# ChangUk/RecommenderSystems

Hardware: AMD Instinct MI355X
Metric: RWR seeds/sec + achieved HBM GB/s on 100M-edge bipartite graph, 1/2/4/8 GPUs (higher is better)
Workload: dtype f64

## Files before the change

### recommendersystems_amd/csrc/iterate.hip

```cpp
#include "iterate.h"

#include <climits>
#include <cstdlib>
#include <type_traits>

namespace rwr {

template <int G, bool VF>
__global__ __launch_bounds__(256) void k_spmm(int32_t n, const int64_t *__restrict__ in_ptr,
                                              const int32_t *__restrict__ in_src,
                                              const double *__restrict__ in_w,
                                              const int32_t *__restrict__ row_order, int32_t nrows,
                                              const double *__restrict__ X, double *__restrict__ Y,
                                              const int32_t *__restrict__ seeds, double c1, int skip_seed_row,
                                              const double *__restrict__ w_src, double *__restrict__ Zout)
{
    constexpr int RPW = WAVE / G;
    constexpr int U = 4;
    const int tile = blockIdx.y;
    const size_t toff = (size_t)tile * (size_t)n * G;
    X += toff;
    Y += toff;
    if (VF && Zout) Zout += toff;
    const int lane = threadIdx.x & (WAVE - 1);
    const int sub = lane / G, k = lane % G;
    const int32_t my_seed = skip_seed_row ? seeds[tile * G + k] : -1;
    const int wpb = blockDim.x / WAVE;
    const int64_t nwaves = (int64_t)gridDim.x * wpb;
    for (int64_t rb = ((int64_t)blockIdx.x * wpb + threadIdx.x / WAVE) * RPW; rb < nrows; rb += nwaves * RPW) {
        const int64_t r = rb + sub;
        int32_t j = -1;
        int64_t p = 0, e = 0;
        if (r < nrows) {
            j = row_order[r];
            p = in_ptr[j];
            e = in_ptr[j + 1];
        }
        double acc = 0.0;
        for (; p + U <= e; p += U) {
            int32_t idx[U];
            double wv[U], xv[U];
#pragma unroll
            for (int u = 0; u < U; ++u) idx[u] = in_src[p + u];
#pragma unroll
            for (int u = 0; u < U; ++u) wv[u] = VF ? 0.0 : in_w[p + u];
#pragma unroll
            for (int u = 0; u < U; ++u) xv[u] = X[(size_t)idx[u] * G + k];
#pragma unroll
            for (int u = 0; u < U; ++u) {
                if (VF) {
                    acc += xv[u];
                } else {
                    double rw = c1 * xv[u];
                    acc += rw * wv[u];
                }
            }
        }
        for (; p < e; ++p) {
            if (VF) {
                acc += X[(size_t)in_src[p] * G + k];
            } else {
                double rw = c1 * X[(size_t)in_src[p] * G + k];
                acc += rw * in_w[p];
            }
        }
        if (j >= 0 && j != my_seed) {
            Y[(size_t)j * G + k] = acc;
            if (VF && Zout) { const double rw = c1 * acc; Zout[(size_t)j * G + k] = rw * w_src[j]; }
        }
    }
}

template <int G, int CH, bool CHECK, bool WRITE, bool VF>
__device__ __forceinline__ void spmm_chunked_body(int32_t n, const int64_t *__restrict__ in_ptr,
                                                  const int32_t *__restrict__ in_src,
                                                  const double *__restrict__ in_w,
                                                  const int32_t *__restrict__ row_order, int32_t nrows,
                                                  const double *__restrict__ X, double *__restrict__ Y,
                                                  const int32_t *__restrict__ seeds, double c1,
                                                  int skip_seed_row, const uint32_t *__restrict__ nz_in,
                                                  uint32_t *__restrict__ nz_out,
                                                  const uint32_t *__restrict__ act,
                                                  const double *__restrict__ w_src, double *__restrict__ Zout)
{
    static_assert(G >= 8 && G <= 64, "chunked SpMM needs 8 <= G <= 64");
    constexpr int RPW = WAVE / G;
    const int tile = blockIdx.y;
    const size_t toff = (size_t)tile * (size_t)n * G;
    X += toff;
    Y += toff;
    if (VF && Zout) Zout += toff;
    const size_t nzw = ((size_t)n + 31) / 32;
    if (CHECK) nz_in += (size_t)tile * nzw;
    if (WRITE) nz_out += (size_t)tile * nzw;
    if (CHECK && act) act += (size_t)tile * nzw;
    const int lane = threadIdx.x & (WAVE - 1);
    const int sub = lane / G, k = lane % G;
    const int gbase = (lane - k) << 2;
    const int32_t my_seed = skip_seed_row ? seeds[tile * G + k] : -1;
    const int wpb = blockDim.x / WAVE;
    const int64_t nwaves = (int64_t)gridDim.x * wpb;
    for (int64_t rb = ((int64_t)blockIdx.x * wpb + threadIdx.x / WAVE) * RPW; rb < nrows; rb += nwaves * RPW) {
        const int64_t r = rb + sub;
        int32_t j = -1;
        int64_t p = 0, e = 0;
        if (r < nrows) {
            j = row_order[r];
            p = in_ptr[j];
            e = in_ptr[j + 1];
            if (CHECK && act && !((act[(uint32_t)j >> 5] >> (j & 31)) & 1u)) e = p;
        }
        double acc = 0.0;
        while (__any(p < e)) {
            const int64_t left = e - p;
            const int cnt = left > CH ? CH : (left > 0 ? (int)left : 0);
            int32_t my_idx = 0;
            double my_w = 0.0;
            if (k < cnt) {
                my_idx = in_src[p + k];
                if (!VF) my_w = in_w[p + k];
                if (CHECK) {
                    const uint32_t wd = nz_in[(uint32_t)my_idx >> 5];
                    if (!((wd >> (my_idx & 31)) & 1u)) my_idx |= (int32_t)0x80000000;
                }
            }
            const int wlo = __double2loint(my_w), whi = __double2hiint(my_w);
            if (CHECK) {
                const unsigned long long lm = __ballot(k < cnt && my_idx >= 0);
                unsigned long long um = lm;
                if (G < 64) {
#pragma unroll
                    for (int sh = G; sh < 64; sh <<= 1) um |= um >> sh;
                    um &= (1ull << (G & 63)) - 1ull;
                }
                if (__popcll(um) <= 4) {
                    while (um) {
                        const int t = __builtin_ctzll(um);
                        um &= um - 1;
                        const int idx = __builtin_amdgcn_ds_bpermute(gbase + (t << 2), my_idx);
                        if (VF) {
                            if (t < cnt && idx >= 0) acc += X[(size_t)idx * G + k];
                        } else {
                            const int lo = __builtin_amdgcn_ds_bpermute(gbase + (t << 2), wlo);
                            const int hi = __builtin_amdgcn_ds_bpermute(gbase + (t << 2), whi);
                            if (t < cnt && idx >= 0) {
                                const double rw = c1 * X[(size_t)idx * G + k];
                                acc += rw * __hiloint2double(hi, lo);
                            }
                        }
                    }
                    p += cnt;
                    continue;
                }
            }
            double xv[CH], wv[CH];
#pragma unroll
            for (int t = 0; t < CH; ++t) {
                const int idx = __builtin_amdgcn_ds_bpermute(gbase + (t << 2), my_idx);
                if (!VF) {
                    const int lo = __builtin_amdgcn_ds_bpermute(gbase + (t << 2), wlo);
                    const int hi = __builtin_amdgcn_ds_bpermute(gbase + (t << 2), whi);
                    wv[t] = __hiloint2double(hi, lo);
                }
                xv[t] = (t < cnt && idx >= 0) ? X[(size_t)idx * G + k] : 0.0;
            }
#pragma unroll
            for (int t = 0; t < CH; ++t) {
                if (t < cnt) {
                    if (VF) {
                        acc += xv[t];
                    } else {
                        double rw = c1 * xv[t];
                        acc += rw * wv[t];
                    }
                }
            }
            p += cnt;
        }
        if (j >= 0 && j != my_seed) {
            Y[(size_t)j * G + k] = acc;
            if (VF && Zout) { const double rw = c1 * acc; Zout[(size_t)j * G + k] = rw * w_src[j]; }
        }
        if (WRITE) {
            const unsigned long long nzb = __ballot(acc != 0.0);
            const unsigned long long gmask = (G == 64) ? ~0ull : (((1ull << (G & 63)) - 1ull) << (sub * G));
            if (k == 0 && j >= 0 && (nzb & gmask)) atomicOr(&nz_out[(uint32_t)j >> 5], 1u << (j & 31));
        }
    }
}

template <int G, int CH, bool CHECK, bool WRITE, bool VF, bool LIST>
__global__ __launch_bounds__(256) void k_spmm_chunked(int32_t n, const int64_t *__restrict__ in_ptr,
                                                      const int32_t *__restrict__ in_src,
                                                      const double *__restrict__ in_w,
                                                      const int32_t *__restrict__ row_order, int32_t nrows,
                                                      const double *__restrict__ X, double *__restrict__ Y,
                                                      const int32_t *__restrict__ seeds, double c1,
                                                      int skip_seed_row, const uint32_t *__restrict__ nz_in,
                                                      uint32_t *__restrict__ nz_out,
                                                      const uint32_t *__restrict__ act,
                                                      const double *__restrict__ w_src, double *__restrict__ Zout)
{
    spmm_chunked_body<G, CH, CHECK, WRITE, VF>(n, in_ptr, in_src, in_w, row_order, nrows, X, Y, seeds, c1, skip_seed_row,
                                               nz_in, nz_out, act, w_src, Zout);
}

template <int G, int CH, bool VF>
__global__ __launch_bounds__(256) void k_spmm_frontier(int32_t n, const int64_t *__restrict__ in_ptr,
                                                       const int32_t *__restrict__ in_src,
                                                       const double *__restrict__ in_w,
                                                       const int32_t *__restrict__ fl_rows,
                                                       const int32_t *__restrict__ fl_cnt,
                                                       const double *__restrict__ X, double *__restrict__ Y,
                                                       const int32_t *__restrict__ seeds, double c1,
                                                       int skip_seed_row, const uint32_t *__restrict__ nz_in,
                                                       uint32_t *__restrict__ nz_out,
                                                       const double *__restrict__ w_src, double *__restrict__ Zout)
{
    const int tile = blockIdx.y;
    spmm_chunked_body<G, CH, true, true, VF>(n, in_ptr, in_src, in_w, fl_rows + (size_t)tile * (size_t)n, fl_cnt[tile], X, Y,
                                             seeds, c1, skip_seed_row, nz_in, nz_out, nullptr, w_src, Zout);
}

__global__ __launch_bounds__(256) void k_mark_active(int32_t n, const uint32_t *__restrict__ nz, uint32_t *__restrict__ act,
                                                     const int64_t *__restrict__ rowptr, const int32_t *__restrict__ dst,
                                                     const uint8_t *__restrict__ etype, int G, const int32_t *__restrict__ seeds,
                                                     int32_t *__restrict__ fl_rows, int32_t *__restrict__ fl_cnt)
{
    const size_t nzw = ((size_t)n + 31) / 32;
    const int tile = blockIdx.y;
    const int lane = threadIdx.x & (WAVE - 1);
    const size_t wi = (size_t)blockIdx.x * (blockDim.x / WAVE) + threadIdx.x / WAVE;
    uint32_t *a = act + (size_t)tile * nzw;
    int32_t *list = fl_rows ? fl_rows + (size_t)tile * (size_t)n : nullptr;
    if (list && blockIdx.x == 0 && threadIdx.x < (unsigned)G) {
        const int32_t sr = seeds[tile * G + threadIdx.x];
        if (sr >= 0) {
            const uint32_t bit = 1u << (sr & 31);
            if (!(atomicOr(&a[(uint32_t)sr >> 5], bit) & bit)) list[atomicAdd(&fl_cnt[tile], 1)] = sr;
        }
    }
    if (wi >= nzw) return;
    uint32_t w = nz[(size_t)tile * nzw + wi];
    while (w) {
        const int b = __builtin_ctz(w);
        w &= w - 1;
        const int64_t i = (int64_t)wi * 32 + b;
        const int64_t p1 = rowptr[i + 1];
        if (!list) {
            for (int64_t p = rowptr[i] + lane; p < p1; p += WAVE)
                if (etype[p] != RWR_EDGE_UNDEFINED) {
                    const int32_t t = dst[p];
                    atomicOr(&a[(uint32_t)t >> 5], 1u << (t & 31));
                }
            continue;
        }
        for (int64_t p0 = rowptr[i]; p0 < p1; p0 += WAVE) {
            const int64_t p = p0 + lane;
            bool add = false;
            int32_t t = 0;
            if (p < p1 && etype[p] != RWR_EDGE_UNDEFINED) {
                t = dst[p];
                const uint32_t bit = 1u << (t & 31);
                add = !(atomicOr(&a[(uint32_t)t >> 5], bit) & bit);
            }
            const unsigned long long m = __ballot(add);
            if (!m) continue;
            const int leader = __builtin_ctzll(m);
            int base = 0;
            if (lane == leader) base = atomicAdd(&fl_cnt[tile], (int)__popcll(m));
            base = __shfl(base, leader);
            const int below = __builtin_amdgcn_mbcnt_hi((uint32_t)(m >> 32), __builtin_amdgcn_mbcnt_lo((uint32_t)m, 0u));
            if (add) list[base + below] = t;
        }
    }
}

template <int G>
__global__ __launch_bounds__(64) void k_seed_chain(int32_t n, int ntiles, const int64_t *__restrict__ in_ptr,
                                                   const int32_t *__restrict__ in_src,
                                                   const double *__restrict__ in_w,
                                                   const uint8_t *__restrict__ dangling,
                                                   const double *__restrict__ X, double *__restrict__ Y,
                                                   const int32_t *__restrict__ seeds, double c1,
                                                   uint32_t *__restrict__ nz_out)
{
    constexpr int U = 8;
    const int q = blockIdx.x * blockDim.x + threadIdx.x;
    if (q >= ntiles * G) return;
    const int tile = q / G, k = q % G;
    const int32_t s = seeds[q];
    if (s < 0) return;
    const double *x = X + (size_t)tile * (size_t)n * G + k;
    int64_t p = in_ptr[s];
    const int64_t e = in_ptr[s + 1];
    int32_t nxt = (p < e) ? in_src[p] : INT_MAX;
    double acc = 0.0;
    int32_t i = 0;
    for (; i + U <= n; i += U) {
        double xv[U];
        uint8_t dg[U];
#pragma unroll
        for (int u = 0; u < U; ++u) xv[u] = x[(size_t)(i + u) * G];
#pragma unroll
        for (int u = 0; u < U; ++u) dg[u] = dangling[i + u];
#pragma unroll
        for (int u = 0; u < U; ++u) {
            double rw = c1 * xv[u];
            while (nxt == i + u) {
                acc += rw * in_w[p];
                ++p;
                nxt = (p < e) ? in_src[p] : INT_MAX;
            }
            acc += dg[u] ? xv[u] : (xv[u] - rw);
        }
    }
    for (; i < n; ++i) {
        double xi = x[(size_t)i * G];
        double rw = c1 * xi;
        while (nxt == i) {
            acc += rw * in_w[p];
            ++p;
            nxt = (p < e) ? in_src[p] : INT_MAX;
        }
        acc += dangling[i] ? xi : (xi - rw);
    }
    Y[(size_t)tile * (size_t)n * G + (size_t)s * G + k] = acc;
    if (nz_out && acc != 0.0)
        atomicOr(&nz_out[(size_t)tile * (((size_t)n + 31) / 32) + ((uint32_t)s >> 5)], 1u << (s & 31));
}

__global__ void k_gate(const unsigned int *__restrict__ gate, unsigned int expected)
{
    const long long t0 = __builtin_amdgcn_s_memrealtime();
    while (__hip_atomic_load(gate, __ATOMIC_RELAXED, __HIP_MEMORY_SCOPE_AGENT) < expected) {
        if (__builtin_amdgcn_s_memrealtime() - t0 > 100000) break;
        __builtin_amdgcn_s_sleep(32);
    }
}

template <int G, bool VF>
__global__ __launch_bounds__(256) void k_seed_terms(int32_t n, const int64_t *__restrict__ in_ptr,
                                                    const int32_t *__restrict__ in_src,
                                                    const double *__restrict__ in_w, const double *__restrict__ X,
                                                    const int32_t *__restrict__ seeds, double c1,
                                                    const int64_t *__restrict__ evoff, double *__restrict__ evterm,
                                                    const uint32_t *__restrict__ nz)
{
    const int slot = blockIdx.y;
    const int32_t s = seeds[slot];
    if (s < 0) return;
    const int tile = slot / G, k = slot % G;
    const double *x = X + (size_t)tile * (size_t)n * G + k;
    const int64_t p0 = in_ptr[s], deg = in_ptr[s + 1] - p0;
    double *out = evterm + evoff[slot];
    if (nz) nz += (size_t)tile * (((size_t)n + 31) / 32);
    for (int64_t q = (int64_t)blockIdx.x * blockDim.x + threadIdx.x; q < deg; q += (int64_t)gridDim.x * blockDim.x) {
        const int32_t i = in_src[p0 + q];
        if (nz && !((nz[(uint32_t)i >> 5] >> (i & 31)) & 1u)) {
            out[q] = 0.0;
        } else if (VF) {
            out[q] = x[(size_t)i * G];
        } else {
            const double rw = c1 * x[(size_t)i * G];
            out[q] = rw * in_w[p0 + q];
        }
    }
}

template <int G>
__global__ __launch_bounds__(64) void k_seed_chain_sparse(int32_t n, const int64_t *__restrict__ in_ptr,
                                                          const int32_t *__restrict__ in_src,
                                                          const uint8_t *__restrict__ dangling,
                                                          const double *__restrict__ X, double *__restrict__ Y,
                                                          const int32_t *__restrict__ seeds, double c1,
                                                          const int64_t *__restrict__ evoff,
                                                          const double *__restrict__ evterm,
                                                          const uint32_t *__restrict__ nz_x, uint32_t *__restrict__ nz_out,
                                                          unsigned int *__restrict__ gate)
{
    if (threadIdx.x == 0 && gate) __hip_atomic_fetch_add(gate, 1u, __ATOMIC_RELAXED, __HIP_MEMORY_SCOPE_AGENT);
    const int tile = blockIdx.x, lane = threadIdx.x;
    const size_t nzw = ((size_t)n + 31) / 32;
    const uint32_t *bits = nz_x + (size_t)tile * nzw;
    const double *x = X + (size_t)tile * (size_t)n * G;
    const bool consumer = lane < G;
    const int k = lane % G;
    int32_t s = -1;
    int64_t p = 0, e = 0;
    const double *termp = evterm;
    if (consumer) {
        s = seeds[tile * G + k];
        if (s >= 0) {
            p = in_ptr[s];
            e = in_ptr[s + 1];
            termp = evterm + evoff[tile * G + k] - p;
        }
    }
    double acc = 0.0;
    for (size_t w0 = 0; w0 < nzw; w0 += WAVE) {
        const uint32_t word = (w0 + lane < nzw) ? bits[w0 + lane] : 0u;
        unsigned long long mask = __ballot(word != 0u);
        while (mask) {
            const int l = __builtin_ctzll(mask);
            mask &= mask - 1;
            uint32_t wv = (uint32_t)__builtin_amdgcn_readlane((int)word, l);
            while (wv) {
                const int b = __builtin_ctz(wv);
                wv &= wv - 1;
                const int32_t i = (int32_t)((w0 + l) * 32 + b);
                if (consumer && s >= 0) {
                    while (p < e && in_src[p] < i) ++p;
                    while (p < e && in_src[p] == i) { acc += termp[p]; ++p; }
                    const double xi = x[(size_t)i * G + k];
                    const double rw = c1 * xi;
                    acc += dangling[i] ? xi : (xi - rw);
                }
            }
        }
    }
    if (consumer && s >= 0) {
        Y[(size_t)tile * (size_t)n * G + (size_t)s * G + k] = acc;
        if (nz_out && acc != 0.0)
            atomicOr(&nz_out[(size_t)tile * nzw + ((uint32_t)s >> 5)], 1u << (s & 31));
    }
}

constexpr int CH3_NSW = 6;
constexpr int CH3_NST = CH3_NSW * WAVE;
constexpr int CH3_LPT = 16;
constexpr int CH3_CE = CH3_NST * CH3_LPT;
template <int G>
__global__ __launch_bounds__(WAVE + CH3_NST) void k_seed_chain_roles(
    int32_t n, const int64_t *__restrict__ in_ptr, const int32_t *__restrict__ in_src,
    const uint8_t *__restrict__ dangling, const double *__restrict__ X, double *__restrict__ Y,
    const int32_t *__restrict__ seeds, double c1, const int64_t *__restrict__ evoff,
    const double *__restrict__ evterm, uint32_t *__restrict__ nz_out, unsigned int *__restrict__ gate)
{
    if (threadIdx.x == 0 && gate) __hip_atomic_fetch_add(gate, 1u, __ATOMIC_RELAXED, __HIP_MEMORY_SCOPE_AGENT);
    constexpr int CR = CH3_CE / G;
    static_assert(CR % 32 == 0, "chunk rows must be a multiple of 32");
    extern __shared__ double rr[];
    const int tile = blockIdx.x;
    const double *x = X + (size_t)tile * (size_t)n * G;
    const int tid = threadIdx.x;
    const int64_t total = (int64_t)n * G;
    const int nchunks = (int)((total + CH3_CE - 1) / CH3_CE);

    if (tid >= WAVE) {
        const int st = tid - WAVE;
        double rega[CH3_LPT], regb[CH3_LPT];
        uint8_t dga[CH3_LPT], dgb[CH3_LPT];
#define CH3_LOAD(R, D, C)                                                       \
    {                                                                           \
        const int64_t base__ = (int64_t)(C) * CH3_CE;                           \
        _Pragma("unroll") for (int u = 0; u < CH3_LPT; ++u) {                   \
            int64_t el = base__ + (int64_t)u * CH3_NST + st;                    \
            el = el < total ? el : total - 1;                                   \
            R[u] = x[el];                                                       \
            D[u] = dangling[el / G];                                            \
        }                                                                       \
    }
#define CH3_STAGE(R, D, C)                                                                              \
    {                                                                                                   \
        const int64_t base__ = (int64_t)(C) * CH3_CE;                                                   \
        double *buf__ = rr + (size_t)((C) & 1) * CH3_CE;                                                \
        _Pragma("unroll") for (int u = 0; u < CH3_LPT; ++u) {                                           \
            const int off = u * CH3_NST + st;                                                           \
            const double xv = (base__ + off < total) ? R[u] : 0.0;   \
            const double rw = c1 * xv;                                                                  \
            buf__[off] = D[u] ? xv : (xv - rw);                                                         \
        }                                                                                               \
    }
        CH3_LOAD(rega, dga, 0)
        if (nchunks > 1) CH3_LOAD(regb, dgb, 1)
        for (int c = 0; c < nchunks; c += 2) {
            CH3_STAGE(rega, dga, c)
            if (c + 2 < nchunks) CH3_LOAD(rega, dga, c + 2)
            __builtin_amdgcn_fence(__ATOMIC_RELEASE, "workgroup", "local");
            __builtin_amdgcn_s_barrier();
            if (c + 1 < nchunks) {
                CH3_STAGE(regb, dgb, c + 1)
                if (c + 3 < nchunks) CH3_LOAD(regb, dgb, c + 3)
                __builtin_amdgcn_fence(__ATOMIC_RELEASE, "workgroup", "local");
                __builtin_amdgcn_s_barrier();
            }
        }
#undef CH3_LOAD
#undef CH3_STAGE
        return;
    }

    const bool consumer = tid < G;
    const int k = tid % G;
    int32_t s = -1;
    int64_t p = 0, e = 0;
    const int32_t *srcp = in_src;
    const double *termp = evterm;
    int32_t nxt = INT_MAX, raw_s = INT_MAX;
    double tcur = 0.0, raw_t = 0.0;
    bool has2 = false;
    if (consumer) {
        s = seeds[tile * G + k];
        if (s >= 0) {
            p = in_ptr[s];
            e = in_ptr[s + 1];
            termp = evterm + evoff[tile * G + k] - p;
            if (p < e) { nxt = srcp[p]; tcur = termp[p]; ++p; }
            if (p < e) { raw_s = srcp[p]; raw_t = termp[p]; has2 = true; ++p; }
        }
    }
    double acc = 0.0;
    __builtin_amdgcn_s_setprio(3);
    for (int c = 0; c < nchunks; ++c) {
        __builtin_amdgcn_s_barrier();
        __builtin_amdgcn_fence(__ATOMIC_ACQUIRE, "workgroup", "local");
        const double *buf = rr + (size_t)(c & 1) * CH3_CE;
        const int64_t row0 = (int64_t)c * CR;
#define CH3_READ(V, R0) _Pragma("unroll") for (int u = 0; u < 32; ++u) V[u] = buf[((R0) + u) * G + k];
#define CH3_FOLD(V, R0)                                                                                     \
    {                                                                                                       \
        const bool evt = __any(consumer && nxt < row0 + (R0) + 32);                                         \
        if (!evt) {                                                                                         \
            _Pragma("unroll") for (int u = 0; u < 32; ++u) acc += V[u];                                     \
        } else {                                                                                            \
            _Pragma("unroll") for (int u = 0; u < 32; ++u) {                                                \
                const int32_t i = (int32_t)(row0 + (R0)) + u;                                               \
                if (__any(consumer && nxt == i)) {                                                          \
                    while (consumer && nxt == i) {                                                          \
                        acc += tcur;                                                                        \
                        nxt = has2 ? raw_s : INT_MAX;  \
                        tcur = raw_t;                                                                       \
                        has2 = p < e;                 \
                        const int64_t pc = has2 ? p : e - 1;                                                \
                        raw_s = srcp[pc];                                                                   \
                        raw_t = termp[pc];                                                                  \
                        p += has2 ? 1 : 0;                                                                  \
                    }                                                                                       \
                }                                                                                           \
                acc += V[u];                            \
            }                                                                                               \
        }                                                                                                   \
    }
        double ra[32], rb[32];
        CH3_READ(ra, 0)
#pragma unroll 1
        for (int r0 = 0; r0 + 64 <= CR; r0 += 64) {
            CH3_READ(rb, r0 + 32)
            CH3_FOLD(ra, r0)
            if (r0 + 64 < CR) CH3_READ(ra, r0 + 64)
            CH3_FOLD(rb, r0 + 32)
        }
        if (CR % 64 != 0) CH3_FOLD(ra, CR - 32)
#undef CH3_READ
#undef CH3_FOLD
    }
    __builtin_amdgcn_s_setprio(0);
    if (consumer && s >= 0) {
        Y[(size_t)tile * (size_t)n * G + (size_t)s * G + k] = acc;
        if (nz_out && acc != 0.0)
            atomicOr(&nz_out[(size_t)tile * (((size_t)n + 31) / 32) + ((uint32_t)s >> 5)], 1u << (s & 31));
    }
}

__global__ void k_init_seeds(int32_t n, int ntiles, int G, double *__restrict__ X,
                             const int32_t *__restrict__ seeds, uint32_t *__restrict__ nz,
                             double *__restrict__ Z = nullptr, const double *__restrict__ w_src = nullptr, double c1 = 0.0)
{
    const int q = blockIdx.x * blockDim.x + threadIdx.x;
    if (q >= ntiles * G) return;
    const int32_t s = seeds[q];
    if (s < 0) return;
    const int tile = q / G;
    const size_t row = (size_t)tile * (size_t)n * G + (size_t)s * G;
    const double rw = c1 * (double)n;
    const double zs = Z ? rw * w_src[s] : 0.0;
    for (int kk = 0; kk < G; ++kk) {
        const bool mine = seeds[tile * G + kk] == s;
        X[row + kk] = mine ? (double)n : 0.0;
        if (Z) Z[row + kk] = mine ? zs : 0.0;
    }
    if (nz) atomicOr(&nz[(size_t)tile * (((size_t)n + 31) / 32) + ((uint32_t)s >> 5)], 1u << (s & 31));
}

__global__ void k_seed_z(int32_t n, int ntiles, int G, const double *__restrict__ Y, double *__restrict__ Z,
                         const int32_t *__restrict__ seeds, const double *__restrict__ w_src, double c1)
{
    const int q = blockIdx.x * blockDim.x + threadIdx.x;
    if (q >= ntiles * G) return;
    const int32_t s = seeds[q];
    if (s < 0) return;
    const size_t at = (size_t)(q / G) * (size_t)n * G + (size_t)s * G + (q % G);
    const double rw = c1 * Y[at];
    Z[at] = rw * w_src[s];
}
__global__ __launch_bounds__(256) void k_make_z(int64_t elems, int G, const double *__restrict__ X, double *__restrict__ Z,
                                                const double *__restrict__ w_src, double c1)
{
    const int64_t q = (int64_t)blockIdx.x * blockDim.x + threadIdx.x;
    if (q >= elems) return;
    const double rw = c1 * X[q];
    Z[q] = rw * w_src[q / G];
}

__global__ __launch_bounds__(256) void k_make_z_nz(int32_t lo, int32_t hi, int G, const double *__restrict__ X, double *__restrict__ Zs,
                                                   const double *__restrict__ w_src, double c1, uint32_t *__restrict__ nz)
{
    const int64_t j = ((int64_t)lo & ~(int64_t)63) + (int64_t)blockIdx.x * blockDim.x + threadIdx.x;
    bool any = false;
    if (j >= lo && j < hi) {
        const double w = w_src[j];
        const size_t at = (size_t)(j - lo) * G;
        for (int k = 0; k < G; ++k) {
            const double xv = X[(size_t)j * G + k];
            const double rw = c1 * xv;
            Zs[at + k] = rw * w;
            any = any || xv != 0.0;
        }
    }
    const unsigned long long m = __ballot(any);
    const int lane = threadIdx.x & (WAVE - 1);
    if (lane == 0 && (uint32_t)m) nz[(uint64_t)j >> 5] = (uint32_t)m;
    if (lane == 32 && (uint32_t)(m >> 32)) nz[(uint64_t)j >> 5] = (uint32_t)(m >> 32);
}


static PlanInput read_plan_knobs()
{
    PlanInput v;
    const char *e;
    if ((e = getenv("RWR_SPMM"))) v.spmm = atoi(e);
    if ((e = RWR_TUNE_ENV("RWR_NZ_ITERS"))) v.nz_iters = atoi(e);
    if ((e = getenv("RWR_ACT_ITERS"))) v.act_iters = atoi(e);
    if ((e = RWR_TUNE_ENV("RWR_ACT_MIN_N"))) v.act_min_n = atol(e);
    if ((e = getenv("RWR_FRONTIER_LIST"))) v.frontier_list = atoi(e);
    if ((e = getenv("RWR_CHAIN"))) v.chain = atoi(e);
    if ((e = RWR_TUNE_ENV("RWR_SCAN_WORK"))) v.scan_work = atof(e);
    if ((e = RWR_TUNE_ENV("RWR_SCAN_SIDE"))) v.scan_side = atoi(e);
    if ((e = RWR_TUNE_ENV("RWR_GATE"))) v.gate = atoi(e);
    if ((e = getenv("RWR_TAIL_ROWS"))) v.tail_rows = atoi(e);
    if ((e = RWR_TUNE_ENV("RWR_CHAIN_SERIAL"))) v.two_streams = atoi(e) == 0;
    return v;
}
static const PlanInput &plan_knobs() { static const PlanInput k = read_plan_knobs(); return k; }

template <class F> static void bool_dispatch(F &&f) { f(); }
template <class F, class... B> static void bool_dispatch(F &&f, bool b, B... bs)
{
    bool_dispatch([&](auto... c) { if (b) f(std::true_type{}, c...); else f(std::false_type{}, c...); }, bs...);
}

template <int G>
static void launch_spmm_g(rwr_graph *g, int tg, const SpmmArgs &a, hipStream_t s)
{
    const bool vf = a.Zin != nullptr;
    const double *GS = vf ? a.Zin : a.X;
    const int skip = a.skip_seed_row;
    constexpr int RPW = WAVE / G;
    constexpr int CH = G > 16 ? 16 : G;
    if constexpr (G >= 8) {
        if (a.rows.kind == Rows::Frontier) {
            const int32_t *fl_rows = g->fl_rows.p, *fl_cnt = g->fl_rows.p + (size_t)tg * (size_t)g->n;
            const unsigned want = cdiv((size_t)g->n / 10 + 1, (size_t)RPW * 4);
            const unsigned gx = want < 1u ? 1u : want < 2048u ? want : 2048u;
            bool_dispatch([&](auto v) {
                hipLaunchKernelGGL((k_spmm_frontier<G, CH, decltype(v)::value>), dim3(gx, tg), dim3(256), 0, s, g->n, g->in_ptr.p,
                                   g->in_src.p, g->in_w.p, fl_rows, fl_cnt, GS, a.Y, a.seeds, a.c1, skip, a.nz_in, a.nz_out,
                                   g->w_src.p, a.Zout);
            }, vf);
            return;
        }
    }
    const bool listed = a.rows.kind == Rows::Tail;
    const int32_t *order = listed ? g->tail_rows[a.rows.level].p : g->row_order.p;
    const int32_t nrows = listed ? g->tail_n[a.rows.level] : g->n;
    unsigned want = cdiv((size_t)nrows, (size_t)RPW * 4);
    unsigned gx = want < 1u ? 1u : want < 8192u ? want : 8192u;
    if constexpr (G == 1) {
        if (tg == 1 && plan_knobs().spmm != 0) {
            launch_spmv_exact(g, a.X, a.Y, a.seeds, a.c1, skip, a.act, a.nz_out, s, a.Zin, a.Zout, a.hub_scan);
            return;
        }
    }
    if constexpr (G >= 8) {
        if (plan_knobs().spmm != 0) {
            bool_dispatch([&](auto chk, auto wr, auto v, auto lst) {
                if constexpr (decltype(chk)::value || !decltype(wr)::value)
                    hipLaunchKernelGGL((k_spmm_chunked<G, CH, decltype(chk)::value, decltype(wr)::value, decltype(v)::value,
                                                       decltype(lst)::value>), dim3(gx, tg), dim3(256), 0, s, g->n, g->in_ptr.p,
                                       g->in_src.p, g->in_w.p, order, nrows, GS, a.Y, a.seeds, a.c1, skip, a.nz_in, a.nz_out,
                                       a.act, g->w_src.p, a.Zout);
            }, a.nz_in != nullptr, a.nz_in && a.nz_out, vf, listed);
            return;
        }
    }
    bool_dispatch([&](auto v) {
        hipLaunchKernelGGL((k_spmm<G, decltype(v)::value>), dim3(gx, tg), dim3(256), 0, s, g->n, g->in_ptr.p, g->in_src.p,
                           g->in_w.p, order, nrows, GS, a.Y, a.seeds, a.c1, skip, g->w_src.p, a.Zout);
    }, vf);
}
void launch_spmm(rwr_graph *g, int G, int tg, const SpmmArgs &a, hipStream_t s)
{
    RWR_DISPATCH_G(G, launch_spmm_g<GG>(g, tg, a, s));
}
void launch_init_seeds(rwr_graph *g, int G, int tg, double *X, const int32_t *seeds, uint32_t *nz, double *Z, double c1,
                       hipStream_t s)
{
    hipLaunchKernelGGL(k_init_seeds, dim3(cdiv((size_t)tg * G, 64)), dim3(64), 0, s, g->n, tg, G, X, seeds, nz, Z, g->w_src.p, c1);
}
void launch_make_z(int64_t elems, int G, const double *X, double *Z, const double *w_src, double c1, hipStream_t s)
{
    hipLaunchKernelGGL(k_make_z, dim3(cdiv((size_t)elems, 256)), dim3(256), 0, s, elems, G, X, Z, w_src, c1);
}
void launch_make_z_nz(rwr_graph *g, int32_t lo, int32_t hi, int G, const double *X, double *Zs, double c1, uint32_t *nz,
                      hipStream_t s)
{
    const int64_t first = (int64_t)lo & ~(int64_t)63;
    hipLaunchKernelGGL(k_make_z_nz, dim3(cdiv((size_t)((int64_t)hi - first), 256)), dim3(256), 0, s, lo, hi, G, X, Zs, g->w_src.p,
                       c1, nz);
}
void launch_mark_active(rwr_graph *g, int G, int tg, const uint32_t *nz, uint32_t *act, const int32_t *seeds, int32_t *fl_rows,
                        int32_t *fl_cnt, hipStream_t s)
{
    const size_t nzw = ((size_t)g->n + 31) / 32;
    hipLaunchKernelGGL(k_mark_active, dim3(cdiv(nzw, 4), tg), dim3(256), 0, s, g->n, nz, act, g->rowptr.p, g->dst.p, g->etype.p,
                       G, seeds, fl_rows, fl_cnt);
}
template <int G>
static void launch_seed_terms(rwr_graph *g, int tg, const double *X, const int32_t *seeds, double c1,
                              const int64_t *evoff, hipStream_t s, const double *Zin, const uint32_t *nz = nullptr)
{
    const unsigned term_blocks = g->max_in_deg > 256 * 8 ? 8u : cdiv((size_t)(g->max_in_deg > 0 ? g->max_in_deg : 1), 256);
    bool_dispatch([&](auto v) {
        hipLaunchKernelGGL((k_seed_terms<G, decltype(v)::value>), dim3(term_blocks, tg * G), dim3(256), 0, s, g->n, g->in_ptr.p,
                           g->in_src.p, g->in_w.p, Zin ? Zin : X, seeds, c1, evoff, g->d_evterm.p, nz);
    }, Zin != nullptr);
}
template <int G>
static void launch_chain(rwr_graph *g, int tg, const double *X, double *Y, const int32_t *seeds, double c1,
                         const int64_t *evoff, uint32_t *nz_out, unsigned int *gate, hipStream_t s,
                         Chain kind, const uint32_t *nz_x)
{
    if (kind == Chain::Sparse) {
        hipLaunchKernelGGL(k_seed_chain_sparse<G>, dim3(tg), dim3(64), 0, s, g->n, g->in_ptr.p, g->in_src.p,
                           g->dangling.p, X, Y, seeds, c1, evoff, g->d_evterm.p, nz_x, nz_out, gate);
        return;
    }
    if (kind == Chain::Roles) {
        constexpr size_t smem = 2 * CH3_CE * sizeof(double);
        (void)hipFuncSetAttribute((const void *)k_seed_chain_roles<G>, hipFuncAttributeMaxDynamicSharedMemorySize, (int)smem);
        hipLaunchKernelGGL(k_seed_chain_roles<G>, dim3(tg), dim3(WAVE + CH3_NST), smem, s, g->n, g->in_ptr.p,
                           g->in_src.p, g->dangling.p, X, Y, seeds, c1, evoff, g->d_evterm.p, nz_out, gate);
        return;
    }
    hipLaunchKernelGGL(k_seed_chain<G>, dim3(cdiv((size_t)tg * G, 64)), dim3(64), 0, s, g->n, tg, g->in_ptr.p,
                       g->in_src.p, g->in_w.p, g->dangling.p, X, Y, seeds, c1, nz_out);
}

int32_t Profile::record(hipEvent_t &e, hipStream_t s)
{
    e = nullptr;
    if (!on) return RWR_OK;
    if (used == pool.size()) { RWR_HIP(hipEventCreate(&e)); pool.push_back(e); }
    e = pool[used++];
    RWR_HIP(hipEventRecord(e, s));
    return RWR_OK;
}
int32_t Profile::end(std::vector<hipEvent_t> &stage, hipEvent_t a, hipStream_t s)
{
    hipEvent_t b; RWR_TRY(record(b, s));
    if (on) stage.insert(stage.end(), {a, b});
    return RWR_OK;
}
int32_t Profile::fold(rwr_graph *g)
{
    auto drain = [&](const std::vector<hipEvent_t> &v, double *acc, bool dense_only) -> int32_t {
        for (size_t i = 0; i + 1 < v.size(); i += 2) {
            float ms = 0.f;
            if (dense_only && !dense[i / 2]) continue;
            RWR_HIP(hipEventElapsedTime(&ms, v[i], v[i + 1]));
            *acc += ms;
        }
        return RWR_OK;
    };
    if (on) {
        RWR_TRY(drain(spmm, &g->stats.spmm_dense_ms, true));
        RWR_TRY(drain(spmm, &g->stats.spmm_ms, false));
        RWR_TRY(drain(chain, &g->stats.chain_ms, false));
        RWR_TRY(drain(rank, &g->stats.rank_ms, false));
        RWR_TRY(drain(iter, &g->stats.iterate_wall_ms, false));
    }
    reset();
    return RWR_OK;
}

int32_t GroupIter::init(bool fresh, bool ranks_nonneg, bool ranking_only)
{
    const int32_t n = g->n;
    hipStream_t s = g->stream;
    const size_t elems = (size_t)tg * (size_t)n * G;
    PlanInput in = plan_knobs();
    in.n = n; in.nnz = g->nnz; in.nonneg = g->nonneg; in.big_n = spmv_big_n(); in.seed_row_kernel = g->opts.seed_row_kernel;
    in.scan_self = chain_scan_self_contained(G); in.G = G; in.tg = tg; in.c1 = c1;
    in.fresh = fresh; in.ranks_nonneg = ranks_nonneg; in.ranking_only = ranking_only;
    cfg = plan_config(in);
    if (fresh) RWR_HIP(hipMemsetAsync(X, 0, elems * sizeof(double), s));
    if (!fresh && Zc) launch_make_z((int64_t)elems, G, X, Zc, g->w_src.p, c1, s);
    const size_t nzw = ((size_t)n + 31) / 32;
    if (cfg.flist && g->fl_rows.ensure((size_t)tg * (size_t)n + (size_t)tg) != RWR_OK) {
        (void)hipGetLastError();
        cfg.flist = false;
    }
    if (fresh && Zc && !cfg.flist) RWR_HIP(hipMemsetAsync(Zc, 0, elems * sizeof(double), s));
    nz_cur = cfg.nz_iters > 0 ? g->d_nz.p : nullptr;
    nz_oth = cfg.nz_iters > 0 ? g->d_nz.p + (size_t)tg * nzw : nullptr;
    if (nz_cur) RWR_HIP(hipMemsetAsync(nz_cur, 0, (size_t)tg * nzw * sizeof(uint32_t), s));
    if (fresh) launch_init_seeds(g, G, tg, X, d_seeds, nz_cur, Zc, c1, s);
    RWR_HIP(hipGetLastError());
    if (cfg.scan) RWR_TRY(chain_scan_prepare(g, G, tg, d_seeds, s));
    if (Zc && G == 1 && tg == 1 && cfg.addends_nonneg) RWR_TRY(sweep_prepare(g));
    if (Zc && cfg.chain_kind == 0 && !cfg.scan) RWR_TRY(ensure_in_w(g));
    return RWR_OK;
}

int32_t GroupIter::step(const StepPlan &p, Profile &prof)
{
    const int32_t n = g->n;
    hipStream_t s = g->stream;
    const size_t nzw = ((size_t)n + 31) / 32;
    constexpr int GATE_SLOTS = 64;
    const uint32_t *nz_in = p.probe ? nz_cur : nullptr;
    uint32_t *nz_out = p.write_bits ? nz_oth : nullptr;
    if (nz_out) RWR_HIP(hipMemsetAsync(nz_out, 0, (size_t)tg * nzw * sizeof(uint32_t), s));
    uint32_t *act = p.mark ? g->d_nz.p + 2 * (size_t)tg * nzw : nullptr;
    const bool listed = p.rows.kind == Rows::Frontier;
    if (act) {
        int32_t *fl_rows = listed ? g->fl_rows.p : nullptr, *fl_cnt = listed ? fl_rows + (size_t)tg * (size_t)n : nullptr;
        RWR_HIP(hipMemsetAsync(act, 0, (size_t)tg * nzw * sizeof(uint32_t), s));
        if (fl_cnt) RWR_HIP(hipMemsetAsync(fl_cnt, 0, (size_t)tg * sizeof(int32_t), s));
        launch_mark_active(g, G, tg, nz_in, act, d_seeds, fl_rows, fl_cnt, s);
    }
    const uint32_t *nz_terms = p.terms_nz ? nz_in : nullptr;
    double *zout = (Zc && p.form_z) ? Zn : nullptr;
    hipStream_t sc = p.chain_side ? g->stream2 : s;
    unsigned int *gate_it = p.gate ? g->d_gate.p + (it % GATE_SLOTS) : nullptr;
    if (p.chain != Chain::None) {
        if (!p.scan()) RWR_DISPATCH_G(G, launch_seed_terms<GG>(g, tg, X, d_seeds, c1, d_evoff, s, Zc, nz_terms));
        if (gate_it) RWR_HIP(hipMemsetAsync(gate_it, 0, sizeof(unsigned int), s));
        if (p.chain_side) { RWR_HIP(hipEventRecord(g->ev_fork, s)); RWR_HIP(hipStreamWaitEvent(sc, g->ev_fork, 0)); }
        if (p.scan() && !(p.chain_self && Zc)) RWR_DISPATCH_G(G, launch_seed_terms<GG>(g, tg, X, d_seeds, c1, d_evoff, sc, Zc, nz_terms));
        hipEvent_t c0; RWR_TRY(prof.record(c0, sc));
        if (p.scan())
            RWR_TRY(chain_scan_step(g, G, tg, X, Y, d_seeds, d_evoff, c1, nz_out, sc, p.chain_self ? Zc : nullptr,
                                    p.chain_self ? zout : nullptr));
        else
            RWR_DISPATCH_G(G, launch_chain<GG>(g, tg, X, Y, d_seeds, c1, d_evoff, nz_out, gate_it, sc, p.chain, nz_in));
        RWR_TRY(prof.end(prof.chain, c0, sc));
        if (p.chain_side) RWR_HIP(hipEventRecord(g->ev_join, sc));
    }
    if (gate_it) hipLaunchKernelGGL(k_gate, dim3(1), dim3(1), 0, s, gate_it, (unsigned)(tg < 192 ? tg : 192));
    hipEvent_t a; RWR_TRY(prof.record(a, s));
    SpmmArgs sp;
    sp.X = X, sp.Y = Y, sp.seeds = d_seeds, sp.c1 = c1, sp.skip_seed_row = true;
    sp.nz_in = nz_in, sp.nz_out = nz_out, sp.act = act, sp.Zin = Zc, sp.Zout = zout;
    sp.hub_scan = cfg.addends_nonneg, sp.rows = p.rows;
    launch_spmm(g, G, tg, sp, s);
    RWR_TRY(prof.end(prof.spmm, a, s));
    if (prof.on) prof.dense.push_back(p.dense());
    if (p.dense()) { g->stats.spmm_dense_launches += 1; ++dense_steps; }
    if (p.chain_side) RWR_HIP(hipStreamWaitEvent(s, g->ev_join, 0));
    if (zout && p.seed_z) hipLaunchKernelGGL(k_seed_z, dim3(cdiv((size_t)tg * G, 64)), dim3(64), 0, s, n, tg, G, Y, zout, d_seeds, g->w_src.p, c1);
    RWR_HIP(hipGetLastError());
    { double *t = X; X = Y; Y = t; }
    { double *t = Zc; Zc = Zn; Zn = t; }
    { uint32_t *tz = nz_cur; nz_cur = nz_oth; nz_oth = tz; }
    g->stats.spmm_launches += 1;
    g->stats.chain_launches += p.chain != Chain::None; g->stats.frontier_list_launches += listed;
    ++it;
    return RWR_OK;
}

int32_t iterate_group(rwr_graph *g, int G, int tg, const int32_t *d_seeds, const int64_t *d_evoff, const int32_t *h_seeds,
                      double d, int64_t T, Profile &prof, double **final_X, int64_t *dense_steps)
{
    GroupIter gi(g, G, tg, d_seeds, d_evoff, d);
    RWR_TRY(gi.init(true, true, true));
    if (gi.cfg.tails) {
        RWR_TRY(tail_rows_prepare(g));
        gi.cfg.tail_depth = g->tail_depth;
        for (size_t q = 0; q < (size_t)tg * G; ++q)
            if (h_seeds[q] >= 0) gi.cfg.need |= g->h_tail_flag[h_seeds[q]];
    }
    while (gi.it < T) RWR_TRY(gi.step(plan_step(gi.cfg, gi.it, T), prof));
    *final_X = gi.X;
    *dense_steps = gi.dense_steps;
    return RWR_OK;
}

}
```

### recommendersystems_amd/csrc/step_plan.h

```cpp
#pragma once

#include <cstdint>

namespace rwr {

struct PlanInput {
    int spmm = 1, nz_iters = 4, act_iters = -1, frontier_list = 1, chain = 1;
    int64_t act_min_n = 200000; double scan_work = 10000.0;
    int scan_side = 1, gate = 1, tail_rows = 1;
    bool two_streams = true;
    int32_t n = 0, big_n = 2000000;
    int64_t nnz = 0; bool nonneg = true;
    int seed_row_kernel = 0;
    bool scan_self = false;
    int G = 1, tg = 1;
    double c1 = 0.85;
    bool fresh = true;
    bool ranks_nonneg = true;
    bool ranking_only = false;
};

struct PlanConfig {
    int G = 1, tg = 1; bool fresh = true;
    int nz_iters = 0;
    int act_iters = 0;
    bool flist = false;
    bool addends_nonneg = false;
    bool scan = false;
    int chain_kind = 1;
    bool scan_side = false, scan_self = false;
    bool two_streams = true, gate = true;
    bool tails = false; int tail_depth = 0;
    unsigned need = 0;
};

inline PlanConfig plan_config(const PlanInput &in)
{
    PlanConfig c;
    c.G = in.G, c.tg = in.tg, c.fresh = in.fresh;
    const bool single = in.G == 1 && in.tg == 1;
    c.nz_iters = (in.G >= 8 && in.spmm != 0 && in.nonneg) ? in.nz_iters : 0;
    c.act_iters = in.act_iters >= 0 ? in.act_iters : ((in.nnz / (in.n > 0 ? in.n : 1)) <= 64 ? 2 : 1);
    if (single && in.act_iters < 0 && c.act_iters == 2 && in.n >= in.big_n) c.act_iters = 3;
    if (single && in.spmm != 0 && in.nonneg) c.nz_iters = c.act_iters;
    if (single && in.act_iters < 0 && in.n < in.act_min_n) c.nz_iters = c.act_iters = 0;
    if (!in.fresh) c.nz_iters = c.act_iters = 0;
    c.flist = in.ranking_only && in.fresh && in.frontier_list != 0 && in.G >= 8 && c.nz_iters >= 2 && c.act_iters >= 1;
    c.chain_kind = in.seed_row_kernel == 1 ? 3 : in.seed_row_kernel == 2 ? 2 : in.seed_row_kernel == 3 ? 0 : in.chain;
    const double per_seed = 0.89 * (double)in.nnz / (double)(in.n > 0 ? in.n : 1) + 6.7;
    c.addends_nonneg = in.c1 >= 0.0 && in.c1 <= 1.0 && in.nonneg && in.ranks_nonneg;
    c.scan = c.addends_nonneg && (c.chain_kind == 2 || (c.chain_kind == 1 && (double)in.tg * in.G * per_seed < in.scan_work));
    c.scan_side = in.scan_side != 0 && single && in.two_streams && in.n >= 100000;
    c.scan_self = in.scan_self, c.two_streams = in.two_streams, c.gate = in.gate != 0;
    c.tails = in.ranking_only && in.tail_rows != 0 && !single;
    return c;
}

enum class Rows : uint8_t { All, Frontier, Tail };
struct RowSource { Rows kind = Rows::All; int level = 0; };
enum class Chain : uint8_t { None, Scan, ScanSide, Sparse, Roles, Simple };

struct StepPlan {
    RowSource rows;
    bool probe = false, write_bits = false;
    bool mark = false;
    bool terms_nz = false;
    Chain chain = Chain::None;
    bool chain_side = false, gate = false;
    bool chain_self = false;
    bool form_z = false, seed_z = false;
    bool dense() const { return !probe && rows.kind == Rows::All; }
    bool scan() const { return chain == Chain::Scan || chain == Chain::ScanSide; }
};

inline int last_tail(const PlanConfig &c)
{
    for (int k = 0; c.tails && k < c.tail_depth; ++k)
        if ((c.need >> k) & 1u) return k;
    return c.tails ? c.tail_depth - 1 : -1;
}

inline StepPlan plan_step(const PlanConfig &c, int64_t it, int64_t T)
{
    StepPlan p;
    const int64_t k = T - 1 - it;
    const bool last = T >= 0 && k == 0, tail = T >= 0 && k <= last_tail(c);
    p.probe = it < c.nz_iters;
    p.write_bits = it + 1 < c.nz_iters;
    p.mark = p.probe && it < c.act_iters;
    p.terms_nz = c.flist && p.probe;
    if (tail)
        p.rows = {Rows::Tail, (int)k};
    else if (c.flist && T >= 0 && !last && p.mark && p.write_bits && (it + 1 < c.act_iters || it == 1))
        p.rows = {Rows::Frontier, 0};
    if (tail && !((c.need >> k) & 1u)) p.chain = Chain::None;
    else if (c.scan && (!p.mark || c.G == 1)) p.chain = c.scan_side ? Chain::ScanSide : Chain::Scan;
    else if (p.mark) p.chain = Chain::Sparse;
    else p.chain = c.chain_kind == 0 ? Chain::Simple : Chain::Roles;
    const bool fold = p.chain != Chain::None && !p.scan();
    p.chain_side = p.chain == Chain::ScanSide || (fold && c.two_streams);
    p.gate = fold && c.two_streams && c.gate;
    p.chain_self = p.scan() && c.scan_self;
    p.form_z = !last;
    p.seed_z = p.form_z && p.chain != Chain::None && !p.chain_self;
    return p;
}

}
```

Measured before the change: 773.6.

## Compact live edges per wave in probe SpMM before gathering X

Adds a compacted SpMM row path for the probed (nonzero-checked) iterations. Each group tests edge sources against the nonzero bitmap, packs the live edges to the front of the group with ds_permute, and gathers X only for those, using a narrower batch when few remain. It also prefetches the next chunk of indices and weights while the current one is processed. The aim is to cut wasted gathers and divergence on sparse frontiers, at the cost of extra cross-lane permutes; the old chunked path stays available through RWR_PROBE_COMPACT=0.

```diff
diff --git a/recommendersystems_amd/csrc/iterate.hip b/recommendersystems_amd/csrc/iterate.hip
--- a/recommendersystems_amd/csrc/iterate.hip
+++ b/recommendersystems_amd/csrc/iterate.hip
@@ -1,4 +1,5 @@
 #include "iterate.h"
+#include "probe_compact.h"
 
 #include <climits>
 #include <cstdlib>
@@ -71,7 +72,88 @@
     }
 }
 
-template <int G, int CH, bool CHECK, bool WRITE, bool VF>
+template <int G, int CH, bool VF>
+__device__ __forceinline__ double spmm_row_compacted(int64_t p, const int64_t e, const int lane,
+                                                     const int32_t *__restrict__ in_src, const double *__restrict__ in_w,
+                                                     const uint32_t *__restrict__ nz_in, const double *__restrict__ X,
+                                                     const double c1)
+{
+    const int sub = lane / G, k = lane % G;
+    const int gbase = (lane - k) << 2;
+    double acc = 0.0;
+    const unsigned long long gmask = pc_group_mask(G, sub);
+    auto fetch_cnt = [&]() { const int64_t left = e - p; return left > G ? G : (left > 0 ? (int)left : 0); };
+    int cnt = fetch_cnt();
+    int32_t nx_idx = 0;
+    double nx_w = 0.0;
+    if (k < cnt) {
+        nx_idx = in_src[p + k];
+        if (!VF) nx_w = in_w[p + k];
+    }
+    while (__any(p < e)) {
+        const int32_t my_idx = nx_idx;
+        const double my_w = nx_w;
+        const int cur = cnt;
+        p += cur;
+        cnt = fetch_cnt();
+        nx_idx = 0, nx_w = 0.0;
+        if (k < cnt) {
+            nx_idx = in_src[p + k];
+            if (!VF) nx_w = in_w[p + k];
+        }
+        bool live = false;
+        if (k < cur) live = (nz_in[(uint32_t)my_idx >> 5] >> (my_idx & 31)) & 1u;
+        const unsigned long long lm = __ballot(live);
+        if (!lm) continue;
+        const unsigned long long gm = lm & gmask;
+        const int L = pc_live(gm);
+        const int to = gbase + (pc_slot_of(live, pc_rank(gm, lane), k, L) << 2);
+        const int cidx = __builtin_amdgcn_ds_permute(to, my_idx);
+        int clo = 0, chi = 0;
+        if (!VF) {
+            clo = __builtin_amdgcn_ds_permute(to, __double2loint(my_w));
+            chi = __builtin_amdgcn_ds_permute(to, __double2hiint(my_w));
+        }
+        auto batch = [&](auto width, int b0) {
+            constexpr int W = decltype(width)::value;
+            double xv[W], wv[W];
+#pragma unroll
+            for (int t = 0; t < W; ++t) {
+                const int sl = pc_read_slot(b0, t);
+                const int idx = __builtin_amdgcn_ds_bpermute(gbase + (sl << 2), cidx);
+                if (!VF) {
+                    const int lo = __builtin_amdgcn_ds_bpermute(gbase + (sl << 2), clo);
+                    const int hi = __builtin_amdgcn_ds_bpermute(gbase + (sl << 2), chi);
+                    wv[t] = __hiloint2double(hi, lo);
+                }
+                xv[t] = sl < L ? X[(size_t)idx * G + k] : 0.0;
+            }
+#pragma unroll
+            for (int t = 0; t < W; ++t) {
+                if (pc_read_slot(b0, t) < L) {
+                    if (VF) {
+                        acc += xv[t];
+                    } else {
+                        double rw = c1 * xv[t];
+                        acc += rw * wv[t];
+                    }
+                }
+            }
+        };
+        for (int b0 = 0; __any(b0 < L);) {
+            if (CH > PC_SMALL && !__any(b0 + PC_SMALL < L)) {
+                batch(std::integral_constant<int, PC_SMALL>{}, b0);
+                b0 += PC_SMALL;
+            } else {
+                batch(std::integral_constant<int, CH>{}, b0);
+                b0 += CH;
+            }
+        }
+    }
+    return acc;
+}
+
+template <int G, int CH, bool CHECK, bool WRITE, bool VF, bool COMPACT = true>
 __device__ __forceinline__ void spmm_chunked_body(int32_t n, const int64_t *__restrict__ in_ptr,
                                                   const int32_t *__restrict__ in_src,
                                                   const double *__restrict__ in_w,
@@ -111,6 +193,10 @@
             if (CHECK && act && !((act[(uint32_t)j >> 5] >> (j & 31)) & 1u)) e = p;
         }
         double acc = 0.0;
+        if constexpr (CHECK && COMPACT && pc_enabled(G)) {
+            acc = spmm_row_compacted<G, CH, VF>(p, e, lane, in_src, in_w, nz_in, X, c1);
+            p = e;
+        }
         while (__any(p < e)) {
             const int64_t left = e - p;
             const int cnt = left > CH ? CH : (left > 0 ? (int)left : 0);
@@ -220,6 +306,38 @@
     const int tile = blockIdx.y;
     spmm_chunked_body<G, CH, true, true, VF>(n, in_ptr, in_src, in_w, fl_rows + (size_t)tile * (size_t)n, fl_cnt[tile], X, Y,
                                              seeds, c1, skip_seed_row, nz_in, nz_out, nullptr, w_src, Zout);
+}
+
+template <int G, int CH, bool WRITE, bool VF>
+__global__ __launch_bounds__(256) void k_spmm_probe_chunks(int32_t n, const int64_t *__restrict__ in_ptr,
+                                                           const int32_t *__restrict__ in_src,
+                                                           const double *__restrict__ in_w,
+                                                           const int32_t *__restrict__ row_order, int32_t nrows,
+                                                           const double *__restrict__ X, double *__restrict__ Y,
+                                                           const int32_t *__restrict__ seeds, double c1,
+                                                           int skip_seed_row, const uint32_t *__restrict__ nz_in,
+                                                           uint32_t *__restrict__ nz_out,
+                                                           const uint32_t *__restrict__ act,
+                                                           const double *__restrict__ w_src, double *__restrict__ Zout)
+{
+    spmm_chunked_body<G, CH, true, WRITE, VF, false>(n, in_ptr, in_src, in_w, row_order, nrows, X, Y, seeds, c1, skip_seed_row,
+                                                     nz_in, nz_out, act, w_src, Zout);
+}
+template <int G, int CH, bool VF>
+__global__ __launch_bounds__(256) void k_spmm_frontier_chunks(int32_t n, const int64_t *__restrict__ in_ptr,
+                                                              const int32_t *__restrict__ in_src,
+                                                              const double *__restrict__ in_w,
+                                                              const int32_t *__restrict__ fl_rows,
+                                                              const int32_t *__restrict__ fl_cnt,
+                                                              const double *__restrict__ X, double *__restrict__ Y,
+                                                              const int32_t *__restrict__ seeds, double c1,
+                                                              int skip_seed_row, const uint32_t *__restrict__ nz_in,
+                                                              uint32_t *__restrict__ nz_out,
+                                                              const double *__restrict__ w_src, double *__restrict__ Zout)
+{
+    const int tile = blockIdx.y;
+    spmm_chunked_body<G, CH, true, true, VF, false>(n, in_ptr, in_src, in_w, fl_rows + (size_t)tile * (size_t)n, fl_cnt[tile], X,
+                                                    Y, seeds, c1, skip_seed_row, nz_in, nz_out, nullptr, w_src, Zout);
 }
 
 __global__ __launch_bounds__(256) void k_mark_active(int32_t n, const uint32_t *__restrict__ nz, uint32_t *__restrict__ act,
@@ -634,6 +752,7 @@
     if ((e = getenv("RWR_ACT_ITERS"))) v.act_iters = atoi(e);
     if ((e = RWR_TUNE_ENV("RWR_ACT_MIN_N"))) v.act_min_n = atol(e);
     if ((e = getenv("RWR_FRONTIER_LIST"))) v.frontier_list = atoi(e);
+    if ((e = getenv("RWR_PROBE_COMPACT"))) v.probe_compact = atoi(e);
     if ((e = getenv("RWR_CHAIN"))) v.chain = atoi(e);
     if ((e = RWR_TUNE_ENV("RWR_SCAN_WORK"))) v.scan_work = atof(e);
     if ((e = RWR_TUNE_ENV("RWR_SCAN_SIDE"))) v.scan_side = atoi(e);
@@ -663,11 +782,16 @@
             const int32_t *fl_rows = g->fl_rows.p, *fl_cnt = g->fl_rows.p + (size_t)tg * (size_t)g->n;
             const unsigned want = cdiv((size_t)g->n / 10 + 1, (size_t)RPW * 4);
             const unsigned gx = want < 1u ? 1u : want < 2048u ? want : 2048u;
-            bool_dispatch([&](auto v) {
-                hipLaunchKernelGGL((k_spmm_frontier<G, CH, decltype(v)::value>), dim3(gx, tg), dim3(256), 0, s, g->n, g->in_ptr.p,
-                                   g->in_src.p, g->in_w.p, fl_rows, fl_cnt, GS, a.Y, a.seeds, a.c1, skip, a.nz_in, a.nz_out,
-                                   g->w_src.p, a.Zout);
-            }, vf);
+            bool_dispatch([&](auto v, auto chunks) {
+                if constexpr (decltype(chunks)::value && pc_enabled(G))
+                    hipLaunchKernelGGL((k_spmm_frontier_chunks<G, CH, decltype(v)::value>), dim3(gx, tg), dim3(256), 0, s, g->n,
+                                       g->in_ptr.p, g->in_src.p, g->in_w.p, fl_rows, fl_cnt, GS, a.Y, a.seeds, a.c1, skip, a.nz_in,
+                                       a.nz_out, g->w_src.p, a.Zout);
+                else
+                    hipLaunchKernelGGL((k_spmm_frontier<G, CH, decltype(v)::value>), dim3(gx, tg), dim3(256), 0, s, g->n,
+                                       g->in_ptr.p, g->in_src.p, g->in_w.p, fl_rows, fl_cnt, GS, a.Y, a.seeds, a.c1, skip, a.nz_in,
+                                       a.nz_out, g->w_src.p, a.Zout);
+            }, vf, plan_knobs().probe_compact == 0);
             return;
         }
     }
@@ -684,6 +808,14 @@
     }
     if constexpr (G >= 8) {
         if (plan_knobs().spmm != 0) {
+            if (a.nz_in && plan_knobs().probe_compact == 0 && pc_enabled(G)) {
+                bool_dispatch([&](auto wr, auto v) {
+                    hipLaunchKernelGGL((k_spmm_probe_chunks<G, CH, decltype(wr)::value, decltype(v)::value>), dim3(gx, tg),
+                                       dim3(256), 0, s, g->n, g->in_ptr.p, g->in_src.p, g->in_w.p, order, nrows, GS, a.Y, a.seeds,
+                                       a.c1, skip, a.nz_in, a.nz_out, a.act, g->w_src.p, a.Zout);
+                }, a.nz_out != nullptr, vf);
+                return;
+            }
             bool_dispatch([&](auto chk, auto wr, auto v, auto lst) {
                 if constexpr (decltype(chk)::value || !decltype(wr)::value)
                     hipLaunchKernelGGL((k_spmm_chunked<G, CH, decltype(chk)::value, decltype(wr)::value, decltype(v)::value,
diff --git a/recommendersystems_amd/csrc/probe_compact.h b/recommendersystems_amd/csrc/probe_compact.h
--- /dev/null
+++ b/recommendersystems_amd/csrc/probe_compact.h
@@ -0,0 +1,48 @@
+#pragma once
+
+#include <cstdint>
+
+#if defined(__HIPCC__)
+#define RWR_PC_FN __host__ __device__ inline
+#else
+#define RWR_PC_FN inline
+#endif
+
+namespace rwr {
+
+constexpr int PC_WAVE = 64;
+constexpr int PC_SMALL = 4;
+
+RWR_PC_FN constexpr bool pc_enabled(int G) { return G >= 16 && G <= 64; }
+
+RWR_PC_FN constexpr uint64_t pc_group_mask(int G, int sub)
+{
+    return G >= 64 ? ~0ull : (((1ull << G) - 1ull) << (sub * G));
+}
+
+RWR_PC_FN int pc_rank(uint64_t gm, int lane)
+{
+#if defined(__HIP_DEVICE_COMPILE__)
+    (void)lane;
+    return (int)__builtin_amdgcn_mbcnt_hi((uint32_t)(gm >> 32), __builtin_amdgcn_mbcnt_lo((uint32_t)gm, 0u));
+#else
+    return __builtin_popcountll(gm & ((1ull << lane) - 1ull));
+#endif
+}
+
+RWR_PC_FN int pc_live(uint64_t gm) { return __builtin_popcountll(gm); }
+
+RWR_PC_FN constexpr int pc_slot_of(bool live, int rank, int k, int L) { return live ? rank : L + (k - rank); }
+
+RWR_PC_FN constexpr int pc_batch_width(int b0, int Lmax, int CH) { return Lmax - b0 <= PC_SMALL && PC_SMALL < CH ? PC_SMALL : CH; }
+
+RWR_PC_FN constexpr int pc_batches(int Lmax, int CH)
+{
+    int nb = 0;
+    for (int b0 = 0; b0 < Lmax; b0 += pc_batch_width(b0, Lmax, CH)) ++nb;
+    return nb;
+}
+
+RWR_PC_FN constexpr int pc_read_slot(int b0, int t) { return b0 + t; }
+
+}
diff --git a/recommendersystems_amd/csrc/step_plan.h b/recommendersystems_amd/csrc/step_plan.h
--- a/recommendersystems_amd/csrc/step_plan.h
+++ b/recommendersystems_amd/csrc/step_plan.h
@@ -7,7 +7,7 @@
 struct PlanInput {
     int spmm = 1, nz_iters = 4, act_iters = -1, frontier_list = 1, chain = 1;
     int64_t act_min_n = 200000; double scan_work = 10000.0;
-    int scan_side = 1, gate = 1, tail_rows = 1;
+    int scan_side = 1, gate = 1, tail_rows = 1, probe_compact = 1;
     bool two_streams = true;
     int32_t n = 0, big_n = 2000000;
     int64_t nnz = 0; bool nonneg = true;
```

Result: no change. 779.3 (median of 6 runs) (+0.7%).
